# DeepRec-AI/HybridBackend

Hardware: AMD Instinct MI355X
Metric: M-lookups/sec, 26-col Criteo-shape dim16, 1/2/4/8 GPUs; % HBM roofline (higher is better)
Workload: dtype f32

## Files before the change

hybridbackend_amd/csrc/lookup_bwd.hip:

```cpp
#include <alloca.h>
#include <stdlib.h>
#include <string.h>

#include <algorithm>
#include <map>
#include <type_traits>
#include <mutex>
#include <vector>

#include "lookup_common.h"

#ifndef HBK_BWD_WAVES
#define HBK_BWD_WAVES 4
#endif

namespace hbk {
size_t det_sort_temp_bytes(size_t n, int end_bit);
int det_sort_pairs(void* temp, size_t temp_bytes, const uint64_t* keys_in, uint64_t* keys_out,
                   const uint32_t* vals_in, uint32_t* vals_out, size_t n, int end_bit,
                   hipStream_t stream);
size_t det_scan_temp_bytes(size_t n);
int det_scan(void* temp, size_t temp_bytes, const int32_t* in, int32_t* out, size_t n,
             hipStream_t stream);
namespace {

constexpr int kBlock = 256;
constexpr int kWavesPerBlock = kBlock / kWave;
constexpr int kMaxCols = 64;
#ifndef HBK_BWD_TILE
#define HBK_BWD_TILE 2048
#endif
constexpr int kTile = HBK_BWD_TILE;
constexpr int kPerThread = kTile / kBlock;
constexpr int kBatch = kPerThread < 8 ? kPerThread : 8;
constexpr int kMaxBuckets = 16384;
#ifndef HBK_BWD_TEAM
#define HBK_BWD_TEAM 256
#endif
constexpr int kTeam = HBK_BWD_TEAM;
constexpr int kTeams = kBlock / kTeam;
constexpr int kCP = 2 * kTeam;
#ifndef HBK_BWD_RS_CAP
#define HBK_BWD_RS_CAP 2048
#endif
constexpr int kRsCap = HBK_BWD_RS_CAP;
#ifndef HBK_BWD_SLOTX
#define HBK_BWD_SLOTX 2
#endif
constexpr int kSlots = HBK_BWD_SLOTX * kCP;
constexpr int kRoom = kSlots - kTeam - 8;
static_assert(kTeam == 64 || kTeam == kBlock, "a team is one wave or the whole workgroup");

__device__ inline void team_sync() {
  if (kTeam == kBlock) {
    __syncthreads();
  } else {
    __builtin_amdgcn_fence(__ATOMIC_RELEASE, "workgroup");
    __builtin_amdgcn_wave_barrier();
    __builtin_amdgcn_fence(__ATOMIC_ACQUIRE, "workgroup");
  }
}
#ifndef HBK_BWD_PRE
#define HBK_BWD_PRE 3
#endif
constexpr int kPre = HBK_BWD_PRE;
#ifndef HBK_BWD_WIDE_W
#define HBK_BWD_WIDE_W 5
#endif
constexpr int kLdsRowPairs = kCP / 8;
#ifndef HBK_BWD_HOT
#define HBK_BWD_HOT 4
#endif
constexpr int kHotTries = HBK_BWD_HOT;
constexpr int kHotMin = 8;
constexpr unsigned long long kEmptyKey = ~0ull;
constexpr int64_t kDonePair = -1;
constexpr uint16_t kNoSlot = 0xffff;

#ifdef HBK_BWD_STAMPS
constexpr int kTraceBlocks = 8192, kTraceSlots = 8;
__device__ unsigned long long g_bwd_trace[kTraceBlocks * kTraceSlots];
__device__ unsigned long long g_bwd_sub[kTraceBlocks * 4];
#define HBK_SUBSTAMP(i)                                                                    \
  do {                                                                                     \
    if (threadIdx.x == 0 && blockIdx.x < kTraceBlocks) {                                   \
      g_bwd_sub[blockIdx.x * 4 + (i)] = __builtin_amdgcn_s_memrealtime();                  \
    }                                                                                      \
  } while (0)
#define HBK_STAMP_BEGIN()                                                                  \
  if (threadIdx.x == 0 && blockIdx.x < kTraceBlocks) {                                     \
// ... 79 lines not shown
  int32_t merge0[kMaxCols];
  int32_t scan0[kMaxCols];
  int32_t segtile0[kMaxCols];
  int32_t xcd_w;
  int32_t stage_p;
  int32_t xcd_start[10][9];
  GCol col[kMaxCols];
};
static_assert(sizeof(GArgs) <= 24576, "kernarg budget");
static_assert(kMaxCols <= kWave, "one lane per column in HBK_FIND_COL");
static_assert(kSlots <= 65536 && kCP <= 65536, "16-bit LDS indices");

#define HBK_FIND_COL(ARGS, FIELD)                                                  \
  int ci;                                                                          \
  {                                                                                \
    const int l__ = (int)threadIdx.x & (kWave - 1);                                \
    const int v__ = l__ < (ARGS).n_cols ? (ARGS).FIELD[l__] : 0x7fffffff;          \
    ci = (int)__builtin_popcountll(__ballot(v__ <= (int)blockIdx.x)) - 1;          \
    ci = __builtin_amdgcn_readfirstlane(ci);                                       \
  }                                                                                \
  const auto& c = (ARGS).col[ci];

__device__ inline uint32_t mix32(uint64_t row) {
  uint32_t k = (uint32_t)row ^ ((uint32_t)(row >> 32) * 0x9e3779b1u);
  k ^= k >> 16;
  k *= 0x85ebca6bu;
  k ^= k >> 13;
  k *= 0xc2b2ae35u;
  k ^= k >> 16;
  return k;
}

__device__ inline int bucket_of(const GCol& c, uint64_t row) {
  if (c.dense_mul != 0) return (int)__umulhi((uint32_t)row, c.dense_mul);
  return (int)__umulhi(mix32(row), (uint32_t)c.n_buckets);
}

struct RunCursor {
  int k = -1;
  int64_t next = 0;
  int64_t id_delta = 0;
  int64_t grad_delta = 0;
};

__device__ inline void run_seek(const GCol& c, int64_t j, RunCursor& rc) {
  while (j >= rc.next) {
    ++rc.k;
    const int64_t start = c.run_start[rc.k];
    rc.next = rc.k + 1 < c.n_runs ? c.run_start[rc.k + 1] : (int64_t)1 << 62;
    rc.id_delta = c.run_ids[rc.k] - start;
    rc.grad_delta = c.run_grads[rc.k] - start * c.dim;
  }
}

template <typename V>
__device__ inline void scale_segments(const GCol& c, const float* grad, int32_t stride, int combiner,
                                      int64_t s0, int n, const int32_t* sp) {
  constexpr int VE = sizeof(V) / 4;
  constexpr int kU = 4;
  const int tid = (int)threadIdx.x;
  const int sub = tid & ((1 << c.lpr_log2) - 1);
  const int groups = kBlock >> c.lpr_log2;
  if (sub >= c.chunks) return;
  for (int s = tid >> c.lpr_log2; s < n; s += kU * groups) {
    V g[kU];
    int32_t len[kU];
#pragma unroll
    for (int u = 0; u < kU; ++u) {
      const int ss = s + u * groups < n ? s + u * groups : n - 1;
      len[u] = s + u * groups < n ? sp[ss + 1] - sp[ss] : 0;
      g[u] = __builtin_nontemporal_load(reinterpret_cast<const V*>(
          grad + (s0 + ss) * (int64_t)stride + (int64_t)sub * VE));
    }
#pragma unroll
    for (int u = 0; u < kU; ++u) {
      if (len[u] <= 0) continue;
      const V v = combiner == HBK_COMBINER_MEAN ? g[u] / (float)len[u]
                                                : g[u] / sqrtf((float)len[u]);
      *reinterpret_cast<V*>(c.scaled + (s0 + s + u * groups) * (int64_t)c.dim + (int64_t)sub * VE) = v;
    }
  }
}

__device__ inline int32_t seg_search_wave(const int32_t* splits, int64_t n_seg, int32_t j) {
  const int lane = (int)threadIdx.x & (kWave - 1);
  int64_t lo = 0, n = n_seg;
  while (n > 1) {
    const int64_t step = (n + kWave - 1) / kWave;
    const int64_t s = lo + (int64_t)lane * step;
    const bool le = s < lo + n && splits[s] <= j;
    int k = (int)__builtin_popcountll(__ballot(le));
    if (k < 1) k = 1;
    const int64_t nlo = lo + (int64_t)(k - 1) * step;
    const int64_t rest = lo + n - nlo;
    lo = nlo;
    n = rest < step ? rest : step;
  }
  return (int32_t)lo;
}

__device__ inline int32_t tile_segments(const GCol& c, int64_t j_first, int64_t j_last,
                                        int32_t* seg_lds, int32_t* ends) {
  static_assert(kTile == kBlock * kPerThread && kPerThread % 4 == 0, "whole int4 per thread");
  const int tid = (int)threadIdx.x, lane = tid & (kWave - 1), wave = tid >> 6;
  if (wave == 0) {
    const int32_t s = seg_search_wave(c.splits, c.n_seg, (int32_t)j_first);
    if (tid == 0) ends[0] = s;
  } else if (wave == 1) {
    const int32_t s = seg_search_wave(c.splits, c.n_seg, (int32_t)j_last);
    if (tid == kWave) ends[1] = s;
  }
  int4* const v4 = reinterpret_cast<int4*>(seg_lds) + tid * (kPerThread / 4);
#pragma unroll
  for (int q = 0; q < kPerThread / 4; ++q) v4[q] = make_int4(0, 0, 0, 0);
  __syncthreads();
  const int32_t s_lo = ends[0], s_hi = ends[1];
  for (int32_t s = s_lo + 1 + tid; s <= s_hi; s += kBlock) {
    const int64_t p = (int64_t)c.splits[s] - j_first;
    if (p >= 0 && p < kTile) atomicAdd(&seg_lds[p], 1);
  }
  __syncthreads();
  int32_t x[kPerThread];
#pragma unroll
  for (int q = 0; q < kPerThread / 4; ++q) {
    const int4 v = v4[q];
    x[4 * q] = v.x;
    x[4 * q + 1] = v.y;
    x[4 * q + 2] = v.z;
    x[4 * q + 3] = v.w;
  }
#pragma unroll
  for (int q = 1; q < kPerThread; ++q) x[q] += x[q - 1];
  int32_t incl = x[kPerThread - 1];
#pragma unroll
  for (int o = 1; o < kWave; o <<= 1) {
    const int32_t y = __shfl_up(incl, o, kWave);
    if (lane >= o) incl += y;
  }
  if (lane == kWave - 1) ends[2 + wave] = incl;
  __syncthreads();
  int32_t before = incl - x[kPerThread - 1];
  for (int w = 0; w < wave; ++w) before += ends[2 + w];
#pragma unroll
  for (int q = 0; q < kPerThread / 4; ++q) {
    v4[q] = make_int4(x[4 * q] + before, x[4 * q + 1] + before, x[4 * q + 2] + before,
                      x[4 * q + 3] + before);
  }
  __syncthreads();
  return s_lo;
}

__global__ __launch_bounds__(kBlock) void bwd_segof_kernel(const GArgs a) {
  __shared__ int32_t sp[kBlock + 1];
  HBK_FIND_COL(a, segtile0)
  const int64_t s0 = ((int64_t)blockIdx.x - c.segtile0) * kBlock;
  const int tid = (int)threadIdx.x;
  const int n = c.n_seg - s0 < kBlock ? (int)(c.n_seg - s0) : kBlock;
  if (tid < n) sp[tid] = c.splits[s0 + tid];
  if (tid == 0) sp[n] = c.splits[s0 + n];
  __syncthreads();
  const int32_t lo = sp[0], hi = c.seg_of != nullptr ? sp[n] : sp[0];
  for (int32_t j = lo + tid; j < hi; j += kBlock) {
    int s = 0, e = n;
    while (e - s > 1) {
      const int mid = (s + e) >> 1;
      if (sp[mid] <= j) {
        s = mid;
      } else {
        e = mid;
      }
    }
    c.seg_of[j] = (int32_t)(s0 + s);
  }
  if (c.scaled != nullptr) {
    if (c.vec4) {
      scale_segments<f32x4>(c, c.grad_out, c.grad_stride, c.combiner, s0, n, sp);
    } else {
      scale_segments<float>(c, c.grad_out, c.grad_stride, c.combiner, s0, n, sp);
    }
  }
}

template <bool SIMPLE>
__global__ __launch_bounds__(kBlock) void bwd_hist_kernel(const GArgs a) {
  extern __shared__ int32_t counters[];
  HBK_FIND_COL(a, tile0)
  const int P = c.n_buckets;
  const int tid = (int)threadIdx.x;
  const int ctile = (int)blockIdx.x - c.tile0;
  const int64_t base = (int64_t)ctile * kTile;
  RunCursor rc;
  int64_t id[kBatch];
  auto load_batch = [&](int k0) {
#pragma unroll
    for (int k = 0; k < kBatch; ++k) {
      const int64_t j = base + (int64_t)(k0 + k) * kBlock + tid;
      id[k] = 0;
      if (j < c.n_ids) {
        if (!SIMPLE && c.n_runs > 0) run_seek(c, j, rc);
        id[k] = load_id(c.ids, SIMPLE ? 1 : c.ids64, SIMPLE ? j : j + rc.id_delta);
      }
    }
  };
  load_batch(0);
  for (int p = tid; p < P; p += kBlock) counters[p] = 0;
  __syncthreads();
  for (int k0 = 0; k0 < kPerThread; k0 += kBatch) {
    if (k0 > 0) load_batch(k0);
#pragma unroll
    for (int k = 0; k < kBatch; ++k) {
      const int64_t j = base + (int64_t)(k0 + k) * kBlock + tid;
      if (j < c.n_ids) {
        const uint64_t r = id_to_row(c.map, id[k]);
        if (r != kNoRow) atomicAdd(&counters[SIMPLE ? (int)__umulhi((uint32_t)r, c.dense_mul) : bucket_of(c, r)], 1);
      }
    }
  }
  __syncthreads();
  for (int p = tid; p < P; p += kBlock) c.hist[(int64_t)ctile * P + p] = counters[p];
  if (c.scaled != nullptr) {
    __shared__ int32_t sp[kBlock + 1];
    const int64_t n_tiles = (c.n_ids + kTile - 1) / kTile;
    const int64_t per = (c.n_seg + n_tiles - 1) / n_tiles;
    const int64_t s_begin = (int64_t)ctile * per;
    const int64_t s_end = s_begin + per < c.n_seg ? s_begin + per : c.n_seg;
    for (int64_t s0 = s_begin; s0 < s_end; s0 += kBlock) {
      const int n = s_end - s0 < kBlock ? (int)(s_end - s0) : kBlock;
      __syncthreads();
      if (tid < n) sp[tid] = c.splits[s0 + tid];
      if (tid == 0) sp[n] = c.splits[s0 + n];
      __syncthreads();
// ... 101 lines not shown
__global__ __launch_bounds__(kBlock) void bwd_scan_fused_kernel(const GArgs a) {
  __shared__ int32_t wave_tot[kWavesPerBlock];
  __shared__ int32_t n_extra;
  const GCol& c = a.col[blockIdx.x];
  for (int p = (int)threadIdx.x; p < c.n_buckets; p += kBlock) scan_tiles_of_bucket(c, p);
  __syncthreads();
  scan_buckets_of_column(c, wave_tot, &n_extra);
}

constexpr int kXcdScatterBit = 30;

__global__ __launch_bounds__(kBlock) void bwd_scatter_pairs_kernel(const GArgs a) {
  extern __shared__ int32_t run[];
  const int blk = xcd_contiguous((int)blockIdx.x, (int)gridDim.x, (a.xcd >> kXcdScatterBit) & 1);
  int ci;
  {
    const int l__ = (int)threadIdx.x & (kWave - 1);
    const int v__ = l__ < a.n_cols ? a.tile0[l__] : 0x7fffffff;
    ci = (int)__builtin_popcountll(__ballot(v__ <= blk)) - 1;
    ci = __builtin_amdgcn_readfirstlane(ci);
  }
  const GCol& c = a.col[ci];
  const int P = c.n_buckets;
  const int tid = (int)threadIdx.x;
  const int ctile = blk - c.tile0;
  const int64_t base = (int64_t)ctile * kTile;
  __shared__ int32_t sp_lds[kTile];
  __shared__ int32_t seg_ends[2 + kWavesPerBlock];
  const bool seg_inline = c.splits != nullptr && c.seg_of == nullptr;
  int32_t s_lo = 0;
  if (seg_inline) {
    const int64_t j_last = (base + kTile < c.n_ids ? base + kTile : c.n_ids) - 1;
    s_lo = tile_segments(c, base, j_last, sp_lds, seg_ends);
  }
  RunCursor rc;
  int64_t id[kBatch];
  int32_t seg[kBatch];
  auto load_batch = [&](int k0) {
#pragma unroll
    for (int k = 0; k < kBatch; ++k) {
      const int64_t j = base + (int64_t)(k0 + k) * kBlock + tid;
      id[k] = 0;
      seg[k] = (int32_t)j;
      if (j < c.n_ids) {
        if (c.n_runs > 0) {
          run_seek(c, j, rc);
          if (!c.det) seg[k] = (int32_t)(uint32_t)(rc.grad_delta + j * c.dim);
        }
        id[k] = load_id(c.ids, c.ids64, j + rc.id_delta);
        if (c.seg_of != nullptr) {
          seg[k] = c.seg_of[j];
        } else if (seg_inline) {
          seg[k] = s_lo + sp_lds[(k0 + k) * kBlock + tid];
        }
      }
    }
  };
  load_batch(0);
  for (int p = tid; p < P; p += kBlock) run[p] = c.bstart[p] + c.hist[(int64_t)ctile * P + p];
  __syncthreads();
  for (int k0 = 0; k0 < kPerThread; k0 += kBatch) {
    if (k0 > 0) load_batch(k0);
#pragma unroll
    for (int k = 0; k < kBatch; ++k) {
      const int64_t j = base + (int64_t)(k0 + k) * kBlock + tid;
      if (j < c.n_ids) {
        const uint64_t r = id_to_row(c.map, id[k]);
        if (r != kNoRow) {
          const int32_t pos = atomicAdd(&run[bucket_of(c, r)], 1);
          if (c.packed) {
            c.pair_row[0][pos] = (int64_t)((r << 32) | (uint64_t)(uint32_t)seg[k]);
          } else {
            c.pair_row[0][pos] = (int64_t)r;
            c.pair_seg[0][pos] = seg[k];
          }
        }
      }
    }
  }
}

constexpr int kStageMaxBuckets = 1024;

template <bool SIMPLE>
__global__ __launch_bounds__(kBlock, 4) void bwd_scatter_staged_kernel(const GArgs a) {
  extern __shared__ int32_t stage_dyn[];
  int32_t* const counters = stage_dyn;
  int32_t* const first = stage_dyn + a.stage_p;
  int32_t* const st_seg = stage_dyn + 2 * a.stage_p;
  __shared__ int64_t st_row[kTile];
  __shared__ uint16_t st_b[SIMPLE ? 1 : kTile];
  __shared__ int32_t wave_cnt[kWavesPerBlock];
  __shared__ int32_t n_staged;
  const int blk = xcd_contiguous((int)blockIdx.x, (int)gridDim.x, (a.xcd >> kXcdScatterBit) & 1);
  int ci;
  {
    const int l__ = (int)threadIdx.x & (kWave - 1);
    const int v__ = l__ < a.n_cols ? a.tile0[l__] : 0x7fffffff;
    ci = (int)__builtin_popcountll(__ballot(v__ <= blk)) - 1;
    ci = __builtin_amdgcn_readfirstlane(ci);
  }
  const GCol& c = a.col[ci];
  const int P = c.n_buckets;
  const int tid = (int)threadIdx.x, lane = tid & (kWave - 1), wave = tid >> 6;
  const int ctile = blk - c.tile0;
  const int64_t base = (int64_t)ctile * kTile;
  __shared__ int32_t seg_ends[2 + kWavesPerBlock];
  int32_t* const sp_lds = reinterpret_cast<int32_t*>(st_row);
  const bool seg_inline = c.splits != nullptr && (SIMPLE || c.seg_of == nullptr);
  RunCursor rc;
  int64_t id[kPerThread];
  int32_t seg[kPerThread];
#pragma unroll
  for (int k = 0; k < kPerThread; ++k) {
    const int64_t j = base + (int64_t)k * kBlock + tid;
    id[k] = 0;
    seg[k] = (int32_t)j;
    if (j < c.n_ids) {
      if (!SIMPLE && c.n_runs > 0) {
        run_seek(c, j, rc);
        if (!c.det) seg[k] = (int32_t)(uint32_t)(rc.grad_delta + j * c.dim);
      }
      id[k] = load_id(c.ids, SIMPLE ? 1 : c.ids64, SIMPLE ? j : j + rc.id_delta);
      if (!SIMPLE && c.seg_of != nullptr) seg[k] = c.seg_of[j];
    }
  }
  const int per = (P + kBlock - 1) / kBlock;
  const int beg = tid * per;
  const int end = beg + per < P ? beg + per : P;
  int32_t gpos[kStageMaxBuckets / kBlock];
#pragma unroll
  for (int q = 0; q < kStageMaxBuckets / kBlock; ++q) {
    const int p = beg + q;
    gpos[q] = q < per && p < end ? c.bstart[p] + c.hist[(int64_t)ctile * P + p] : 0;
  }
  if (seg_inline) {
    const int64_t j_last = (base + kTile < c.n_ids ? base + kTile : c.n_ids) - 1;
    const int32_t s_lo = tile_segments(c, base, j_last, sp_lds, seg_ends);
#pragma unroll
    for (int k = 0; k < kPerThread; ++k) seg[k] = s_lo + sp_lds[k * kBlock + tid];
  }
  for (int p = tid; p < P; p += kBlock) counters[p] = 0;
  __syncthreads();
  int32_t br[kPerThread];
#pragma unroll
  for (int k = 0; k < kPerThread; ++k) {
    const int64_t j = base + (int64_t)k * kBlock + tid;
    br[k] = -1;
    if (j < c.n_ids) {
      const uint64_t r = id_to_row(c.map, id[k]);
      id[k] = (int64_t)r;
      if (r != kNoRow) {
        const int b = SIMPLE ? (int)__umulhi((uint32_t)r, c.dense_mul) : bucket_of(c, r);
        br[k] = b | (atomicAdd(&counters[b], 1) << 10);
      }
    }
  }
  __syncthreads();
  int32_t sum_c = 0;
#pragma unroll
  for (int q = 0; q < kStageMaxBuckets / kBlock; ++q) {
    if (q < per && beg + q < end) sum_c += counters[beg + q];
  }
  int32_t incl_c = sum_c;
#pragma unroll
  for (int off = 1; off < kWave; off <<= 1) {
    const int32_t w = __shfl_up(incl_c, off, kWave);
    if (lane >= off) incl_c += w;
  }
  if (lane == kWave - 1) wave_cnt[wave] = incl_c;
  __syncthreads();
  int32_t run_c = incl_c - sum_c;
  for (int w = 0; w < wave; ++w) run_c += wave_cnt[w];
#pragma unroll
  for (int q = 0; q < kStageMaxBuckets / kBlock; ++q) {
    const int p = beg + q;
    if (q < per && p < end) {
      const int32_t n_c = counters[p];
      first[p] = run_c;
      counters[p] = gpos[q] - run_c;
      run_c += n_c;
    }
  }
  if (tid == kBlock - 1) n_staged = run_c;
  __syncthreads();
#pragma unroll
  for (int k = 0; k < kPerThread; ++k) {
    if (br[k] >= 0) {
      const int b = br[k] & 1023;
      const int L = first[b] + (br[k] >> 10);
      if (SIMPLE || c.packed) {
        st_row[L] = (int64_t)(((uint64_t)id[k] << 32) | (uint64_t)(uint32_t)seg[k]);
      } else {
        st_row[L] = id[k];
        st_seg[L] = seg[k];
      }
      if (!SIMPLE) st_b[L] = (uint16_t)b;
    }
  }
  __syncthreads();
  const int n_st = n_staged;
#pragma unroll
  for (int k = 0; k < kPerThread; ++k) {
    const int L = k * kBlock + tid;
    if (L < n_st) {
      const int sb = SIMPLE ? (int)__umulhi((uint32_t)((uint64_t)st_row[L] >> 32), c.dense_mul) : (int)st_b[L];
      const int32_t pos = counters[sb] + L;
      c.pair_row[0][pos] = st_row[L];
      if (!SIMPLE && !c.packed) c.pair_seg[0][pos] = st_seg[L];
    }
  }
}

#ifdef HBK_BWD_STAMPS
__device__ unsigned long long g_grp_trace[kTraceBlocks * kTraceSlots];
#define HBK_GSTAMP(i)                                                                       \
  do {                                                                                      \
    if (threadIdx.x == 0 && blockIdx.x < kTraceBlocks) {                                    \
      g_grp_trace[blockIdx.x * kTraceSlots + (i)] = __builtin_amdgcn_s_memrealtime();       \
    }                                                                                       \
  } while (0)
#else
#define HBK_GSTAMP(i)
#endif

constexpr int kGroupMaxBuckets = 2 * kBlock;

struct GSync {
  int32_t* hist;
  int32_t* zero;
  int64_t zero_words;
  SyncWait wait;
};

template <bool SIMPLE>
__global__ __launch_bounds__(kBlock, 4) void bwd_group_kernel(const GArgs a, const GSync y) {
  __shared__ int32_t counters[kGroupMaxBuckets];
  __shared__ int32_t tot_s[kGroupMaxBuckets], pre_s[kGroupMaxBuckets];
  __shared__ int64_t st_row[kTile];
  extern __shared__ int32_t st_seg[];
  __shared__ uint16_t st_b[kTile];
  __shared__ int32_t wave_tot[kWavesPerBlock], wave_cnt[kWavesPerBlock];
  __shared__ int32_t n_extra, gave_up, n_staged;
  const int tid = (int)threadIdx.x, lane = tid & (kWave - 1), wave = tid >> 6;
  HBK_GSTAMP(0);
  for (int64_t j = (int64_t)blockIdx.x * kBlock + tid; j < y.zero_words;
       j += (int64_t)gridDim.x * kBlock) {
    y.zero[j] = 0;
  }
  HBK_FIND_COL(a, tile0)
  const int P = c.n_buckets;
  const int ctile = (int)blockIdx.x - c.tile0;
  const int n_tiles = (int)((c.n_ids + kTile - 1) / kTile);
  const int64_t base = (int64_t)ctile * kTile;
  int32_t* hist = y.hist + c.sync0;
  __shared__ int32_t seg_ends[2 + kWavesPerBlock];
  int32_t* const sp_lds = reinterpret_cast<int32_t*>(st_row);
  const bool seg_inline = c.splits != nullptr && (SIMPLE || c.seg_of == nullptr);
  RunCursor rc;
  int64_t id[kPerThread];
  int32_t seg[kPerThread];
#pragma unroll
  for (int k = 0; k < kPerThread; ++k) {
    const int64_t j = base + (int64_t)k * kBlock + tid;
    id[k] = 0;
    seg[k] = (int32_t)j;
    if (j < c.n_ids) {
      if (!SIMPLE && c.n_runs > 0) {
        run_seek(c, j, rc);
        if (!c.det) seg[k] = (int32_t)(uint32_t)(rc.grad_delta + j * c.dim);
      }
      id[k] = load_id(c.ids, SIMPLE ? 1 : c.ids64, SIMPLE ? j : j + rc.id_delta);
      if (!SIMPLE && c.seg_of != nullptr) seg[k] = c.seg_of[j];
    }
  }
  if (seg_inline) {
    const int64_t j_last = (base + kTile < c.n_ids ? base + kTile : c.n_ids) - 1;
    const int32_t s_lo = tile_segments(c, base, j_last, sp_lds, seg_ends);
#pragma unroll
    for (int k = 0; k < kPerThread; ++k) seg[k] = s_lo + sp_lds[k * kBlock + tid];
  }
  for (int p = tid; p < P; p += kBlock) counters[p] = 0;
  if (tid == 0) {
    n_extra = 0;
    gave_up = 0;
  }
  __syncthreads();
  HBK_GSTAMP(1);
  int32_t br[kPerThread];
#pragma unroll
  for (int k = 0; k < kPerThread; ++k) {
    const int64_t j = base + (int64_t)k * kBlock + tid;
    br[k] = -1;
// ... 2758 lines not shown
  for (int32_t i = 0; i < g.k; ++i) {
    g_ids += cols[members[i]].n_ids;
    g_bytes += (int64_t)cols[members[i]].n_ids * cols[members[i]].dim * 4;
    ++by_kind[info[(size_t)members[i]].kind];
  }
  fprintf(stderr, "[hbk bwd] group %d on stream %d: %d columns (%s), %lld ids, %.1f MB of gradient rows, "
          "%lld tiles, %lld job slots; columns by kind", group_no, stream_no, g.k,
          g.onepass ? "one-launch" : "large", (long long)g_ids, (double)g_bytes / 1e6, (long long)g.tiles,
          (long long)g.buckets);
  for (int q = 0; q < kKinds; ++q) {
    if (by_kind[q] != 0) fprintf(stderr, " %d:%d", q, by_kind[q]);
  }
  fprintf(stderr, "\n");
}

void place_xcds(Group& g) {
  GArgs& args = g.args;
  args.xcd = 0;
  for (int kind = 0; kind < kKinds; ++kind) {
    if (!g.have_kind[kind] || options().bwd_xcd == 0) continue;
    bool even = options().bwd_xcd == 2;
    if (!even) {
      const int64_t per = slots_per_block(kind);
      const int64_t n = (g.slot_hi[kind] - g.slot_lo[kind] + per - 1) / per;
      const int64_t q = n / 8, r = n % 8;
      double work[8] = {0}, total = 0;
      int64_t slot = 0;
      int x = 0;
      int64_t x_end = (r > 0 ? q + 1 : q) * per;
      for (const KindCol& kc : g.kind_cols[kind]) {
        for (int part = 0; part < 2; ++part) {
          int64_t len = part == 0 ? kc.n_buckets : kc.e_max;
          const double w = part == 0 ? (double)kc.weight : 0.0;
          while (len > 0) {
            while (x < 7 && slot >= x_end) {
              ++x;
              x_end += (x < r ? q + 1 : q) * per;
            }
            const int64_t take = x < 7 && x_end - slot < len ? x_end - slot : len;
            work[x] += w * (double)take;
            total += w * (double)take;
            slot += take;
            len -= take;
          }
        }
      }
      double heaviest = 0;
      for (double w : work) heaviest = w > heaviest ? w : heaviest;
      even = total > 0 && heaviest <= 1.08 * total / 8;
    }
    if (even) args.xcd |= 1 << kind;
  }
  args.xcd_w = 0;
  if ((options().bwd_xcd == 4 || options().bwd_xcd == 1 || options().bwd_xcd == 3) && kTeams == 1) {
    for (int kind = 0; kind < kKinds; ++kind) {
      if (!g.have_kind[kind]) continue;
      if (options().bwd_xcd != 4 && !((args.xcd >> kind) & 1)) continue;
      double total = 0;
      for (const KindCol& kc : g.kind_cols[kind]) total += (double)kc.weight * kc.n_buckets;
      if (total <= 0) continue;
      int32_t* st = args.xcd_start[kind];
      st[0] = 0;
      int x = 1;
      double acc = 0;
      int64_t slot = 0;
      for (const KindCol& kc : g.kind_cols[kind]) {
        for (int64_t b = 0; b < kc.n_buckets; ++b) {
          while (x < 8 && acc >= total * x / 8) st[x++] = (int32_t)(slot + b);
          acc += kc.weight;
        }
        slot += (int64_t)kc.n_buckets + kc.e_max;
      }
      while (x <= 8) st[x++] = (int32_t)slot;
      st[8] = (int32_t)(g.slot_hi[kind] - g.slot_lo[kind]);
      int64_t longest = 0;
      for (int q = 0; q < 8; ++q) longest = st[q + 1] - st[q] > longest ? st[q + 1] - st[q] : longest;
      g.xcd_grid[kind] = 8 * longest;
      args.xcd_w |= 1 << kind;
    }
  }
  if (options().bwd_xcd == 1 || options().bwd_xcd == 2) args.xcd |= 1 << kXcdScatterBit;
}

bool launch_grouping(Group& g, hipStream_t ls, hipStream_t caller, GSync* sync) {
  GArgs& args = g.args;
  const int32_t k = g.k;
  const dim3 tiles((unsigned)g.tiles), block(kBlock);
  if (g.ks > 0) {
    g.seg_args.n_cols = g.ks;
    g.seg_args.lr = 0.f;
    hipLaunchKernelGGL(bwd_segof_kernel, dim3((unsigned)g.segtiles), block, 0, ls, g.seg_args);
  }
  bool simple_group = options().bwd_simple != 0;
  bool unpacked = false;
  for (int32_t i = 0; i < k; ++i) {
    const GCol& c = args.col[i];
    simple_group = simple_group && c.n_runs == 0 && c.seg_of == nullptr && c.packed != 0 && c.ids64 != 0 &&
                   c.dense_mul != 0;
    unpacked = unpacked || c.packed == 0;
  }
  const size_t lds_tail = (unpacked ? (size_t)kTile * 4 : 0) + (size_t)options().bwd_lds_pad * 1024;
  memset(sync, 0, sizeof(*sync));
  const auto group_kernel = simple_group ? &bwd_group_kernel<true> : &bwd_group_kernel<false>;
  bool onepass = g.onepass && g.sync_words < (1ll << 30);
  if (onepass) {
    SyncTake take;
    onepass = sync_take(ls, (size_t)g.sync_words, &take, reinterpret_cast<const void*>(group_kernel), kBlock,
                        64, caller);
    if (onepass) {
      sync->hist = take.words;
      sync->zero = take.zero;
      sync->zero_words = take.zero_words;
      sync->wait = sync_wait_of(take);
    }
  }
  if (onepass) {
    SyncChain chain(ls);
    hipLaunchKernelGGL(group_kernel, tiles, block, lds_tail, ls, args, *sync);
    return true;
  }
  hipLaunchKernelGGL(simple_group ? &bwd_hist_kernel<true> : &bwd_hist_kernel<false>, tiles, block, g.lds_hist,
                     ls, args);
  if (g.small_scan) {
    hipLaunchKernelGGL(bwd_scan_fused_kernel, dim3((unsigned)k), block, 0, ls, args);
  } else {
    hipLaunchKernelGGL(bwd_scan_tiles_kernel, dim3((unsigned)g.scans), block, 0, ls, args);
    hipLaunchKernelGGL(bwd_scan_kernel, dim3((unsigned)k), block, 0, ls, args);
  }
  if (g.lds_hist <= (size_t)4 * kStageMaxBuckets && options().bwd_scatter_staged != 0) {
    args.stage_p = (int32_t)(g.lds_hist / 4);
    hipLaunchKernelGGL(simple_group ? &bwd_scatter_staged_kernel<true> : &bwd_scatter_staged_kernel<false>,
                       tiles, block, 2 * g.lds_hist + lds_tail, ls, args);
  } else {
    hipLaunchKernelGGL(bwd_scatter_pairs_kernel, tiles, block, g.lds_hist, ls, args);
  }
  return false;
}

int launch_reduce_merge(const Group& g, bool det, int32_t apply, float apply_lr, const int4* desc,
                        const int32_t* poison, hipStream_t ls) {
  const GArgs& args = g.args;
  const int step = apply_lr == 0.0f ? 0 : apply == HBK_APPLY_ADAGRAD ? 2 : 1;
  typedef void (*reduce_fn)(const GArgs, const int4*, int, int, const int32_t*);
  typedef void (*merge_fn)(const GArgs, int, const int32_t*);
#define HBK_BY_STEP(K, V, ...) {&K<V, 0, ##__VA_ARGS__>, &K<V, 1, ##__VA_ARGS__>, &K<V, 2, ##__VA_ARGS__>}
  static const reduce_fn kReduce[kKinds][3] = {
      HBK_BY_STEP(bwd_dense_kernel, f32x4, false), HBK_BY_STEP(bwd_dense_kernel, float, false),
      HBK_BY_STEP(bwd_dense_kernel, f32x4, true), HBK_BY_STEP(bwd_dense_kernel, float, true),
      HBK_BY_STEP(bwd_reduce_kernel, f32x4, false), HBK_BY_STEP(bwd_reduce_kernel, float, false),
      {nullptr, &bwd_reduce_kernel<f32x4, 1, true>, &bwd_reduce_kernel<f32x4, 2, true>},
      {nullptr, &bwd_reduce_kernel<float, 1, true>, &bwd_reduce_kernel<float, 2, true>},
      HBK_BY_STEP(bwd_rowsort_kernel, f32x4), HBK_BY_STEP(bwd_rowsort_kernel, float)};
  static const merge_fn kMerge[kKinds][3] = {
      HBK_BY_STEP(bwd_dense_merge_kernel, f32x4), HBK_BY_STEP(bwd_dense_merge_kernel, float),
      HBK_BY_STEP(bwd_dense_merge_kernel, f32x4), HBK_BY_STEP(bwd_dense_merge_kernel, float),
      HBK_BY_STEP(bwd_merge_kernel, f32x4, false), HBK_BY_STEP(bwd_merge_kernel, float, false),
      {nullptr, &bwd_merge_kernel<f32x4, 1, true>, &bwd_merge_kernel<f32x4, 2, true>},
      {nullptr, &bwd_merge_kernel<float, 1, true>, &bwd_merge_kernel<float, 2, true>},
      HBK_BY_STEP(bwd_rowsort_merge_kernel, f32x4), HBK_BY_STEP(bwd_rowsort_merge_kernel, float)};
  static const reduce_fn kReduceDet[2][3] = {HBK_BY_STEP(bwd_rowsort_kernel, f32x4, true),
                                             HBK_BY_STEP(bwd_rowsort_kernel, float, true)};
#undef HBK_BY_STEP
  int status = HBK_OK;
  if (det) {
    hipLaunchKernelGGL(bwd_rowsort_count_kernel, dim3((unsigned)g.buckets), dim3(kBlock), 0, ls, args, desc,
                       (int)g.buckets, poison);
  }
  for (int kind = 0; kind < kKinds; ++kind) {
    if (!g.have_kind[kind]) continue;
    const int64_t n_slots = g.slot_hi[kind] - g.slot_lo[kind];
    const int64_t per = slots_per_block(kind);
    const int64_t grid = g.xcd_grid[kind] > 0 ? g.xcd_grid[kind] : (n_slots + per - 1) / per;
    if (det && bucket_kind_of(kind) != kRowSorted) {
      status = fail(HBK_INTERNAL, "group_lookup_bwd: a deterministic column without row-sorted buckets");
      break;
    }
    hipLaunchKernelGGL(det ? kReduceDet[kind & 1][step] : kReduce[kind][step],
                       dim3((unsigned)grid), dim3(kBlock), 0, ls, args, desc, (int)g.slot_lo[kind],
                       (int)g.slot_hi[kind], poison);
  }
  for (int kind = 0; kind < kKinds; ++kind) {
    if (!g.have_kind[kind]) continue;
    hipLaunchKernelGGL(kMerge[kind][step], dim3((unsigned)(g.merge_hi[kind] - g.merge_lo[kind])),
                       dim3(kBlock), 0, ls, args, (int)g.merge_lo[kind], poison);
  }
  const hipError_t launch_err = hipGetLastError();
  if (launch_err != hipSuccess) {
    status = fail(HBK_INTERNAL, "group_lookup_bwd: launch failed: %s", hipGetErrorString(launch_err));
  }
  return status;
}

int bwd_planned(int32_t n_cols, const hbk_lookup_grad_column_t* cols, const std::vector<ColInfo>& info,
                int form, int32_t apply, float apply_lr, void* workspace, hipStream_t stream) {
  const bool det = form == kFormInOrder;
  const std::vector<int32_t> order = order_columns(n_cols, cols, info, form);
  const int32_t live_cols = (int32_t)order.size();
  Carve at;
  at.counter = reinterpret_cast<char*>(((uintptr_t)workspace + 255) & ~(uintptr_t)255);
  at.desc = at.counter + (size_t)256 * order.size();
  at.buf = at.desc;
  for (int32_t c : order) at.buf += info[(size_t)c].lay.desc_bytes;
  for (int32_t c = 0; c < n_cols; ++c) {
    if (cols[c].n_ids == 0 && info[(size_t)c].form == form) {
      HBK_HIP_OK(hipMemsetAsync(cols[c].n_unique, 0, sizeof(int32_t), stream));
    }
  }

  int group_cols = options().bwd_group_cols;
  if (group_cols <= 0 || group_cols > kMaxCols) group_cols = kMaxCols;
  bool mixed = false;
  for (int32_t q = 1; q < live_cols; ++q) {
    mixed = mixed || info[(size_t)order[q]].onepass != info[(size_t)order[0]].onepass;
  }
  const int n_streams = options().bwd_streams < 0 ? 0 : options().bwd_streams > kHelperStreams
// ... 180 lines not shown
```

Before: 30090.

## Make staged scatter kernel persistent and overlap next tile's segment search

Converts the staged scatter kernel into a persistent grid, sized from the occupancy API, that loops over tiles, with XCD-aware tile ranges. Inside the loop it interleaves the wave-wide binary search for the next tile's segment bounds with the current tile's bucketing phases, and prefetches the next tile's ids and histogram. It also replaces shfl_up scans with ds_bpermute and keeps rows as 32-bit in the simple path. This aims to hide global-memory latency of the dependent search loads and cut launch and tail overhead, at the cost of more registers, more complex control flow and a host-side occupancy cache.

```diff
diff --git a/hybridbackend_amd/csrc/lookup_bwd.hip b/hybridbackend_amd/csrc/lookup_bwd.hip
--- a/hybridbackend_amd/csrc/lookup_bwd.hip
+++ b/hybridbackend_amd/csrc/lookup_bwd.hip
@@ -6,6 +6,7 @@
 #include <map>
 #include <type_traits>
 #include <mutex>
+#include <tuple>
 #include <vector>
 
 #include "lookup_common.h"
@@ -251,27 +252,97 @@
   }
 }
 
+struct SegSearch {
+  int64_t lo, n;
+  int32_t j;
+  int32_t probe;
+};
+
+__device__ inline void seg_search_probe(const int32_t* splits, SegSearch& q) {
+  if (q.n > 1) {
+    const int lane = (int)threadIdx.x & (kWave - 1);
+    const int64_t step = (q.n + kWave - 1) / kWave;
+    const int64_t s = q.lo + (int64_t)lane * step;
+    q.probe = s < q.lo + q.n ? splits[s] : 0x7fffffff;
+  }
+}
+
+__device__ inline void seg_search_begin(const int32_t* splits, int64_t n_seg, int32_t j, SegSearch& q) {
+  q.lo = 0;
+  q.n = n_seg;
+  q.j = j;
+  q.probe = 0;
+  seg_search_probe(splits, q);
+}
+
+__device__ inline void seg_search_advance(const int32_t* splits, SegSearch& q) {
+  if (q.n > 1) {
+    const int64_t step = (q.n + kWave - 1) / kWave;
+    int k = (int)__builtin_popcountll(__ballot(q.probe <= q.j));
+    if (k < 1) k = 1;
+    const int64_t nlo = q.lo + (int64_t)(k - 1) * step;
+    const int64_t rest = q.lo + q.n - nlo;
+    q.lo = nlo;
+    q.n = rest < step ? rest : step;
+    seg_search_probe(splits, q);
+  }
+}
+
 __device__ inline int32_t seg_search_wave(const int32_t* splits, int64_t n_seg, int32_t j) {
-  const int lane = (int)threadIdx.x & (kWave - 1);
-  int64_t lo = 0, n = n_seg;
-  while (n > 1) {
-    const int64_t step = (n + kWave - 1) / kWave;
-    const int64_t s = lo + (int64_t)lane * step;
-    const bool le = s < lo + n && splits[s] <= j;
-    int k = (int)__builtin_popcountll(__ballot(le));
-    if (k < 1) k = 1;
-    const int64_t nlo = lo + (int64_t)(k - 1) * step;
-    const int64_t rest = lo + n - nlo;
-    lo = nlo;
-    n = rest < step ? rest : step;
-  }
-  return (int32_t)lo;
+  SegSearch q;
+  seg_search_begin(splits, n_seg, j, q);
+  while (q.n > 1) seg_search_advance(splits, q);
+  return (int32_t)q.lo;
+}
+
+__device__ inline int32_t wave_scan_incl(int32_t x, int lane) {
+#pragma unroll
+  for (int o = 1; o < kWave; o <<= 1) {
+    const int32_t y = __builtin_amdgcn_ds_bpermute(((lane - o) & (kWave - 1)) << 2, x);
+    if (lane >= o) x += y;
+  }
+  return x;
+}
+
+template <bool PRE>
+__device__ inline void tile_segments_fill(int tid, const GCol& c, int64_t j_first, int32_t s_lo, int32_t s_hi,
+                                          int32_t split0, int32_t* seg_lds, int32_t* wave_tot) {
+  const int lane = tid & (kWave - 1), wave = tid >> 6;
+  int4* const v4 = reinterpret_cast<int4*>(seg_lds) + tid * (kPerThread / 4);
+  for (int32_t s = s_lo + 1 + tid; s <= s_hi; s += kBlock) {
+    const int32_t start = PRE && s == s_lo + 1 + tid ? split0 : c.splits[s];
+    const int64_t p = (int64_t)start - j_first;
+    if (p >= 0 && p < kTile) atomicAdd(&seg_lds[p], 1);
+  }
+  __syncthreads();
+  int32_t x[kPerThread];
+#pragma unroll
+  for (int q = 0; q < kPerThread / 4; ++q) {
+    const int4 v = v4[q];
+    x[4 * q] = v.x;
+    x[4 * q + 1] = v.y;
+    x[4 * q + 2] = v.z;
+    x[4 * q + 3] = v.w;
+  }
+#pragma unroll
+  for (int q = 1; q < kPerThread; ++q) x[q] += x[q - 1];
+  const int32_t incl = wave_scan_incl(x[kPerThread - 1], lane);
+  if (lane == kWave - 1) wave_tot[wave] = incl;
+  __syncthreads();
+  int32_t before = incl - x[kPerThread - 1];
+  for (int w = 0; w < wave; ++w) before += wave_tot[w];
+#pragma unroll
+  for (int q = 0; q < kPerThread / 4; ++q) {
+    v4[q] = make_int4(x[4 * q] + before, x[4 * q + 1] + before, x[4 * q + 2] + before,
+                      x[4 * q + 3] + before);
+  }
+  __syncthreads();
 }
 
 __device__ inline int32_t tile_segments(const GCol& c, int64_t j_first, int64_t j_last,
                                         int32_t* seg_lds, int32_t* ends) {
   static_assert(kTile == kBlock * kPerThread && kPerThread % 4 == 0, "whole int4 per thread");
-  const int tid = (int)threadIdx.x, lane = tid & (kWave - 1), wave = tid >> 6;
+  const int tid = (int)threadIdx.x, wave = tid >> 6;
   if (wave == 0) {
     const int32_t s = seg_search_wave(c.splits, c.n_seg, (int32_t)j_first);
     if (tid == 0) ends[0] = s;
@@ -283,39 +354,8 @@
 #pragma unroll
   for (int q = 0; q < kPerThread / 4; ++q) v4[q] = make_int4(0, 0, 0, 0);
   __syncthreads();
-  const int32_t s_lo = ends[0], s_hi = ends[1];
-  for (int32_t s = s_lo + 1 + tid; s <= s_hi; s += kBlock) {
-    const int64_t p = (int64_t)c.splits[s] - j_first;
-    if (p >= 0 && p < kTile) atomicAdd(&seg_lds[p], 1);
-  }
-  __syncthreads();
-  int32_t x[kPerThread];
-#pragma unroll
-  for (int q = 0; q < kPerThread / 4; ++q) {
-    const int4 v = v4[q];
-    x[4 * q] = v.x;
-    x[4 * q + 1] = v.y;
-    x[4 * q + 2] = v.z;
-    x[4 * q + 3] = v.w;
-  }
-#pragma unroll
-  for (int q = 1; q < kPerThread; ++q) x[q] += x[q - 1];
-  int32_t incl = x[kPerThread - 1];
-#pragma unroll
-  for (int o = 1; o < kWave; o <<= 1) {
-    const int32_t y = __shfl_up(incl, o, kWave);
-    if (lane >= o) incl += y;
-  }
-  if (lane == kWave - 1) ends[2 + wave] = incl;
-  __syncthreads();
-  int32_t before = incl - x[kPerThread - 1];
-  for (int w = 0; w < wave; ++w) before += ends[2 + w];
-#pragma unroll
-  for (int q = 0; q < kPerThread / 4; ++q) {
-    v4[q] = make_int4(x[4 * q] + before, x[4 * q + 1] + before, x[4 * q + 2] + before,
-                      x[4 * q + 3] + before);
-  }
-  __syncthreads();
+  const int32_t s_lo = ends[0];
+  tile_segments_fill<false>(tid, c, j_first, s_lo, ends[1], 0, seg_lds, ends + 2);
   return s_lo;
 }
 
@@ -583,8 +623,14 @@
 
 constexpr int kStageMaxBuckets = 1024;
 
+__device__ inline void xcd_range(int x, int n, int* first, int* len) {
+  const int q = n >> 3, r = n & 7;
+  *first = x < r ? x * (q + 1) : r * (q + 1) + (x - r) * q;
+  *len = x < r ? q + 1 : q;
+}
+
 template <bool SIMPLE>
-__global__ __launch_bounds__(kBlock, 4) void bwd_scatter_staged_kernel(const GArgs a) {
+__global__ __launch_bounds__(kBlock, 4) void bwd_scatter_staged_kernel(const GArgs a, const int32_t n_tiles) {
   extern __shared__ int32_t stage_dyn[];
   int32_t* const counters = stage_dyn;
   int32_t* const first = stage_dyn + a.stage_p;
@@ -592,124 +638,214 @@
   __shared__ int64_t st_row[kTile];
   __shared__ uint16_t st_b[SIMPLE ? 1 : kTile];
   __shared__ int32_t wave_cnt[kWavesPerBlock];
+  __shared__ int32_t wave_tot[kWavesPerBlock];
   __shared__ int32_t n_staged;
-  const int blk = xcd_contiguous((int)blockIdx.x, (int)gridDim.x, (a.xcd >> kXcdScatterBit) & 1);
-  int ci;
-  {
-    const int l__ = (int)threadIdx.x & (kWave - 1);
-    const int v__ = l__ < a.n_cols ? a.tile0[l__] : 0x7fffffff;
-    ci = (int)__builtin_popcountll(__ballot(v__ <= blk)) - 1;
-    ci = __builtin_amdgcn_readfirstlane(ci);
-  }
-  const GCol& c = a.col[ci];
-  const int P = c.n_buckets;
-  const int tid = (int)threadIdx.x, lane = tid & (kWave - 1), wave = tid >> 6;
-  const int ctile = blk - c.tile0;
-  const int64_t base = (int64_t)ctile * kTile;
-  __shared__ int32_t seg_ends[2 + kWavesPerBlock];
+  __shared__ int32_t seg_lohi[2][2];
+  const int tid0 = (int)threadIdx.x, lane0 = tid0 & (kWave - 1);
+  const int wave_u = __builtin_amdgcn_readfirstlane(tid0 >> 6);
+  int tile, tile_end, tile_step;
+  if ((a.xcd >> kXcdScatterBit) & 1) {
+    const int x = (int)blockIdx.x & 7;
+    int x_first, x_len;
+    xcd_range(x, n_tiles, &x_first, &x_len);
+    tile = x_first + ((int)blockIdx.x >> 3);
+    tile_end = x_first + x_len;
+    tile_step = ((int)gridDim.x - x + 7) >> 3;
+  } else {
+    tile = (int)blockIdx.x;
+    tile_end = n_tiles;
+    tile_step = (int)gridDim.x;
+  }
+  if (tile >= tile_end) return;
+  const int tile0_lane = lane0 < a.n_cols ? a.tile0[lane0] : 0x7fffffff;
+  auto col_of = [&](int t) {
+    return __builtin_amdgcn_readfirstlane((int)__builtin_popcountll(__ballot(tile0_lane <= t)) - 1);
+  };
   int32_t* const sp_lds = reinterpret_cast<int32_t*>(st_row);
-  const bool seg_inline = c.splits != nullptr && (SIMPLE || c.seg_of == nullptr);
-  RunCursor rc;
+  auto inline_of = [&](const GCol& c) { return c.splits != nullptr && (SIMPLE || c.seg_of == nullptr); };
+  auto load_ids = [&](int tid, const GCol& c, int t, int64_t (&id)[kPerThread], int32_t (&seg)[kPerThread]) {
+    const int64_t base = (int64_t)(t - c.tile0) * kTile;
+    RunCursor rc;
+#pragma unroll
+    for (int k = 0; k < kPerThread; ++k) {
+      const int64_t j = base + (int64_t)k * kBlock + tid;
+      if (SIMPLE) {
+        id[k] = load_id(c.ids, 1, j < c.n_ids ? j : c.n_ids - 1);
+        continue;
+      }
+      id[k] = 0;
+      seg[k] = (int32_t)j;
+      if (j < c.n_ids) {
+        if (c.n_runs > 0) {
+          run_seek(c, j, rc);
+          if (!c.det) seg[k] = (int32_t)(uint32_t)(rc.grad_delta + j * c.dim);
+        }
+        id[k] = load_id(c.ids, c.ids64, j + rc.id_delta);
+        if (c.seg_of != nullptr) seg[k] = c.seg_of[j];
+      }
+    }
+  };
+  auto load_hist = [&](int tid, const GCol& c, int t, int32_t (&gpos)[kStageMaxBuckets / kBlock]) {
+    const int ctile = t - c.tile0;
+    const int P = c.n_buckets;
+    const int per = (P + kBlock - 1) / kBlock;
+#pragma unroll
+    for (int q = 0; q < kStageMaxBuckets / kBlock; ++q) {
+      const int p = tid * per + q < P ? tid * per + q : P - 1;
+      gpos[q] = c.hist[(int64_t)ctile * P + p];
+    }
+  };
+  auto search_pos = [&](const GCol& c, int t) {
+    const int64_t base = (int64_t)(t - c.tile0) * kTile;
+    return (int32_t)(wave_u == 0 ? base : (base + kTile < c.n_ids ? base + kTile : c.n_ids) - 1);
+  };
+  auto first_split = [&](int tid, const GCol& c, int slot) {
+    const int32_t s = seg_lohi[slot][0] + 1 + tid;
+    return s <= seg_lohi[slot][1] ? c.splits[s] : 0;
+  };
+  int ci = col_of(tile);
   int64_t id[kPerThread];
   int32_t seg[kPerThread];
-#pragma unroll
-  for (int k = 0; k < kPerThread; ++k) {
-    const int64_t j = base + (int64_t)k * kBlock + tid;
-    id[k] = 0;
-    seg[k] = (int32_t)j;
-    if (j < c.n_ids) {
-      if (!SIMPLE && c.n_runs > 0) {
-        run_seek(c, j, rc);
-        if (!c.det) seg[k] = (int32_t)(uint32_t)(rc.grad_delta + j * c.dim);
-      }
-      id[k] = load_id(c.ids, SIMPLE ? 1 : c.ids64, SIMPLE ? j : j + rc.id_delta);
-      if (!SIMPLE && c.seg_of != nullptr) seg[k] = c.seg_of[j];
-    }
-  }
-  const int per = (P + kBlock - 1) / kBlock;
-  const int beg = tid * per;
-  const int end = beg + per < P ? beg + per : P;
   int32_t gpos[kStageMaxBuckets / kBlock];
-#pragma unroll
-  for (int q = 0; q < kStageMaxBuckets / kBlock; ++q) {
-    const int p = beg + q;
-    gpos[q] = q < per && p < end ? c.bstart[p] + c.hist[(int64_t)ctile * P + p] : 0;
-  }
-  if (seg_inline) {
-    const int64_t j_last = (base + kTile < c.n_ids ? base + kTile : c.n_ids) - 1;
-    const int32_t s_lo = tile_segments(c, base, j_last, sp_lds, seg_ends);
-#pragma unroll
-    for (int k = 0; k < kPerThread; ++k) seg[k] = s_lo + sp_lds[k * kBlock + tid];
-  }
-  for (int p = tid; p < P; p += kBlock) counters[p] = 0;
-  __syncthreads();
-  int32_t br[kPerThread];
-#pragma unroll
-  for (int k = 0; k < kPerThread; ++k) {
-    const int64_t j = base + (int64_t)k * kBlock + tid;
-    br[k] = -1;
-    if (j < c.n_ids) {
-      const uint64_t r = id_to_row(c.map, id[k]);
-      id[k] = (int64_t)r;
-      if (r != kNoRow) {
-        const int b = SIMPLE ? (int)__umulhi((uint32_t)r, c.dense_mul) : bucket_of(c, r);
-        br[k] = b | (atomicAdd(&counters[b], 1) << 10);
-      }
-    }
-  }
-  __syncthreads();
-  int32_t sum_c = 0;
-#pragma unroll
-  for (int q = 0; q < kStageMaxBuckets / kBlock; ++q) {
-    if (q < per && beg + q < end) sum_c += counters[beg + q];
-  }
-  int32_t incl_c = sum_c;
-#pragma unroll
-  for (int off = 1; off < kWave; off <<= 1) {
-    const int32_t w = __shfl_up(incl_c, off, kWave);
-    if (lane >= off) incl_c += w;
-  }
-  if (lane == kWave - 1) wave_cnt[wave] = incl_c;
-  __syncthreads();
-  int32_t run_c = incl_c - sum_c;
-  for (int w = 0; w < wave; ++w) run_c += wave_cnt[w];
-#pragma unroll
-  for (int q = 0; q < kStageMaxBuckets / kBlock; ++q) {
-    const int p = beg + q;
-    if (q < per && p < end) {
-      const int32_t n_c = counters[p];
-      first[p] = run_c;
-      counters[p] = gpos[q] - run_c;
-      run_c += n_c;
-    }
-  }
-  if (tid == kBlock - 1) n_staged = run_c;
-  __syncthreads();
-#pragma unroll
-  for (int k = 0; k < kPerThread; ++k) {
-    if (br[k] >= 0) {
-      const int b = br[k] & 1023;
-      const int L = first[b] + (br[k] >> 10);
-      if (SIMPLE || c.packed) {
-        st_row[L] = (int64_t)(((uint64_t)id[k] << 32) | (uint64_t)(uint32_t)seg[k]);
-      } else {
-        st_row[L] = id[k];
-        st_seg[L] = seg[k];
-      }
-      if (!SIMPLE) st_b[L] = (uint16_t)b;
-    }
-  }
-  __syncthreads();
-  const int n_st = n_staged;
-#pragma unroll
-  for (int k = 0; k < kPerThread; ++k) {
-    const int L = k * kBlock + tid;
-    if (L < n_st) {
-      const int sb = SIMPLE ? (int)__umulhi((uint32_t)((uint64_t)st_row[L] >> 32), c.dense_mul) : (int)st_b[L];
-      const int32_t pos = counters[sb] + L;
-      c.pair_row[0][pos] = st_row[L];
-      if (!SIMPLE && !c.packed) c.pair_seg[0][pos] = st_seg[L];
-    }
+  int32_t split0 = 0;
+  load_ids(tid0, a.col[ci], tile, id, seg);
+  load_hist(tid0, a.col[ci], tile, gpos);
+  if (inline_of(a.col[ci])) {
+    const GCol& c = a.col[ci];
+    if (wave_u < 2) {
+      const int32_t s = seg_search_wave(c.splits, c.n_seg, search_pos(c, tile));
+      if (lane0 == 0) seg_lohi[0][wave_u] = s;
+    }
+    __syncthreads();
+    split0 = first_split(tid0, c, 0);
+  }
+  for (int it = 0;; ++it) {
+    int tid = tid0;
+    asm volatile("" : "+v"(tid));
+    tid &= kBlock - 1;
+    const int lane = tid & (kWave - 1), wave = tid >> 6;
+    const GCol& c = a.col[ci];
+    const int P = c.n_buckets;
+    const int ctile = tile - c.tile0;
+    const int64_t base = (int64_t)ctile * kTile;
+    const bool seg_inline = inline_of(c);
+    const int tile_n = tile + tile_step;
+    const bool more = tile_n < tile_end;
+    const int ci_n = more ? col_of(tile_n) : ci;
+    const GCol& cn = a.col[ci_n];
+    const bool inline_n = more && inline_of(cn);
+    int32_t nsplit0 = 0;
+    SegSearch nq;
+    nq.lo = 0;
+    nq.n = 0;
+    nq.j = 0;
+    nq.probe = 0;
+    if (inline_n && wave_u < 2) seg_search_begin(cn.splits, cn.n_seg, search_pos(cn, tile_n), nq);
+    const int per = (P + kBlock - 1) / kBlock;
+    const int beg = tid * per;
+    const int end = beg + per < P ? beg + per : P;
+    int32_t bst[kStageMaxBuckets / kBlock];
+#pragma unroll
+    for (int q = 0; q < kStageMaxBuckets / kBlock; ++q) bst[q] = c.bstart[beg + q < P ? beg + q : P - 1];
+    int32_t s_lo = 0;
+    if (seg_inline) {
+      int4* const v4 = reinterpret_cast<int4*>(sp_lds) + tid * (kPerThread / 4);
+#pragma unroll
+      for (int q = 0; q < kPerThread / 4; ++q) v4[q] = make_int4(0, 0, 0, 0);
+      __syncthreads();
+      s_lo = seg_lohi[it & 1][0];
+      tile_segments_fill<true>(tid, c, base, s_lo, seg_lohi[it & 1][1], split0, sp_lds, wave_tot);
+    }
+    seg_search_advance(cn.splits, nq);
+    for (int p = tid; p < P; p += kBlock) counters[p] = 0;
+    __syncthreads();
+    int32_t br[kPerThread];
+    uint32_t row32[SIMPLE ? kPerThread : 1];
+#pragma unroll
+    for (int k = 0; k < kPerThread; ++k) {
+      const int64_t j = base + (int64_t)k * kBlock + tid;
+      br[k] = -1;
+      if (j < c.n_ids) {
+        const uint64_t r = id_to_row(c.map, id[k]);
+        if (SIMPLE) {
+          row32[k] = (uint32_t)r;
+        } else {
+          id[k] = (int64_t)r;
+        }
+        if (r != kNoRow) {
+          const int b = SIMPLE ? (int)__umulhi((uint32_t)r, c.dense_mul) : bucket_of(c, r);
+          br[k] = b | (atomicAdd(&counters[b], 1) << 10);
+        }
+      }
+    }
+    __syncthreads();
+    seg_search_advance(cn.splits, nq);
+    int32_t sum_c = 0;
+#pragma unroll
+    for (int q = 0; q < kStageMaxBuckets / kBlock; ++q) {
+      if (q < per && beg + q < end) sum_c += counters[beg + q];
+    }
+    const int32_t incl_c = wave_scan_incl(sum_c, lane);
+    if (lane == kWave - 1) wave_cnt[wave] = incl_c;
+    __syncthreads();
+    int32_t run_c = incl_c - sum_c;
+    for (int w = 0; w < wave; ++w) run_c += wave_cnt[w];
+#pragma unroll
+    for (int q = 0; q < kStageMaxBuckets / kBlock; ++q) {
+      const int p = beg + q;
+      if (q < per && p < end) {
+        const int32_t n_c = counters[p];
+        first[p] = run_c;
+        counters[p] = bst[q] + gpos[q] - run_c;
+        run_c += n_c;
+      }
+    }
+    if (tid == kBlock - 1) n_staged = run_c;
+    if (seg_inline) {
+#pragma unroll
+      for (int k = 0; k < kPerThread; ++k) seg[k] = s_lo + sp_lds[k * kBlock + tid];
+    } else if (SIMPLE) {
+#pragma unroll
+      for (int k = 0; k < kPerThread; ++k) seg[k] = (int32_t)(base + (int64_t)k * kBlock + tid);
+    }
+    while (nq.n > 1) seg_search_advance(cn.splits, nq);
+    if (inline_n && wave_u < 2 && lane == 0) seg_lohi[(it + 1) & 1][wave_u] = (int32_t)nq.lo;
+    __syncthreads();
+    if (inline_n) nsplit0 = first_split(tid, cn, (it + 1) & 1);
+#pragma unroll
+    for (int k = 0; k < kPerThread; ++k) {
+      if (br[k] >= 0) {
+        const int b = br[k] & 1023;
+        const int L = first[b] + (br[k] >> 10);
+        if (SIMPLE || c.packed) {
+          st_row[L] = (int64_t)(((uint64_t)(SIMPLE ? (uint64_t)row32[k] : (uint64_t)id[k]) << 32) | (uint64_t)(uint32_t)seg[k]);
+        } else {
+          st_row[L] = id[k];
+          st_seg[L] = seg[k];
+        }
+        if (!SIMPLE) st_b[L] = (uint16_t)b;
+      }
+    }
+    __syncthreads();
+    if (inline_n) asm volatile("" ::"v"(nsplit0));
+    const int n_st = n_staged;
+#pragma unroll
+    for (int k = 0; k < kPerThread; ++k) {
+      const int L = k * kBlock + tid;
+      if (L < n_st) {
+        const int sb = SIMPLE ? (int)__umulhi((uint32_t)((uint64_t)st_row[L] >> 32), c.dense_mul) : (int)st_b[L];
+        const int32_t pos = counters[sb] + L;
+        c.pair_row[0][pos] = st_row[L];
+        if (!SIMPLE && !c.packed) c.pair_seg[0][pos] = st_seg[L];
+      }
+    }
+    if (!more) break;
+    load_ids(tid, cn, tile_n, id, seg);
+    load_hist(tid, cn, tile_n, gpos);
+    __syncthreads();
+    tile = tile_n;
+    ci = ci_n;
+    split0 = nsplit0;
   }
 }
 
@@ -3634,6 +3770,28 @@
   if (options().bwd_xcd == 1 || options().bwd_xcd == 2) args.xcd |= 1 << kXcdScatterBit;
 }
 
+int64_t scatter_grid(const void* kernel, size_t lds, int64_t tiles) {
+  static std::mutex mu;
+  static std::map<std::tuple<int, const void*, size_t>, int> resident;
+  int dev = 0;
+  (void)hipGetDevice(&dev);
+  int n = 0;
+  {
+    std::lock_guard<std::mutex> lock(mu);
+    const auto key = std::make_tuple(dev, kernel, lds);
+    auto it = resident.find(key);
+    if (it == resident.end()) {
+      int per_cu = 0;
+      if (hipOccupancyMaxActiveBlocksPerMultiprocessor(&per_cu, kernel, kBlock, lds) != hipSuccess || per_cu < 1) {
+        per_cu = 1;
+      }
+      it = resident.emplace(key, per_cu * device_cus()).first;
+    }
+    n = it->second;
+  }
+  return std::min<int64_t>(tiles, std::max(n, 8));
+}
+
 bool launch_grouping(Group& g, hipStream_t ls, hipStream_t caller, GSync* sync) {
   GArgs& args = g.args;
   const int32_t k = g.k;
@@ -3681,8 +3839,10 @@
   }
   if (g.lds_hist <= (size_t)4 * kStageMaxBuckets && options().bwd_scatter_staged != 0) {
     args.stage_p = (int32_t)(g.lds_hist / 4);
-    hipLaunchKernelGGL(simple_group ? &bwd_scatter_staged_kernel<true> : &bwd_scatter_staged_kernel<false>,
-                       tiles, block, 2 * g.lds_hist + lds_tail, ls, args);
+    const auto staged = simple_group ? &bwd_scatter_staged_kernel<true> : &bwd_scatter_staged_kernel<false>;
+    const size_t lds = 2 * g.lds_hist + lds_tail;
+    hipLaunchKernelGGL(staged, dim3((unsigned)scatter_grid(reinterpret_cast<const void*>(staged), lds, g.tiles)),
+                       block, lds, ls, args, (int32_t)g.tiles);
   } else {
     hipLaunchKernelGGL(bwd_scatter_pairs_kernel, tiles, block, g.lds_hist, ls, args);
   }
```

New measurement: 30100 (median of 2 runs). About the same (+0.0%).
